# nju-websoft/OpenEA

Hardware: AMD Instinct MI355X
Metric: training triples/sec (k=10 truncated negatives + limited loss + Adagrad) (higher is better)
Workload: dtype f32; 1 GPU; BootEA/AlignE translational step, EN-FR-100K-V1 shape (synthetic), dim=100, GLOBAL batch=20000 positives (weak scaling: 20000 per GPU x 1 GPU), k=10, truncated eps=0.98; the same workload at every N (; global_batch=20000, entities=200000, parallelism=single

## Files before the change

### openea_amd/csrc/triple_step.hip

```cpp
#include <stdlib.h>

#include <algorithm>
#include <vector>

#include "common.h"
#include "step_plan.h"

namespace {

using oea::group_sum;

using oea::flag_t;
using oea::grad_t;

struct StepWs {
    grad_t *ent_grad, *rel_grad;
    grad_t *rel_extra;
    int64_t rel_copy_stride;
    flag_t *ent_touched, *rel_touched;
    grad_t *nrm_grad, *nrm_extra;
    flag_t *nrm_touched;
    double *partials;
    __device__ __forceinline__ grad_t *rel_copy(int64_t c) const {
        return c == 0 ? rel_grad : rel_extra + (c - 1) * rel_copy_stride;
    }
    __device__ __forceinline__ grad_t *nrm_copy(int64_t c) const {
        return c == 0 ? nrm_grad : nrm_extra + (c - 1) * rel_copy_stride;
    }
};
constexpr int kMaxBlocks = 4096;
constexpr int kRelCopies = 16;

static size_t align256(size_t x) { return (x + 255) / 256 * 256; }

static size_t ws_layout(int64_t n_ent, int64_t n_rel, int32_t ld, void *base, StepWs *ws) {
    size_t off = 0;
    char *b = static_cast<char *>(base);
    auto take = [&](size_t bytes) { size_t o = off; off += align256(bytes); return b ? b + o : nullptr; };
    grad_t *eg = (grad_t *)take(sizeof(grad_t) * (size_t)n_ent * ld);
    grad_t *rg = (grad_t *)take(sizeof(grad_t) * (size_t)n_rel * ld);
    grad_t *ng = (grad_t *)take(sizeof(grad_t) * (size_t)n_rel * ld);
    flag_t *et = (flag_t *)take(sizeof(flag_t) * (size_t)n_ent);
    flag_t *rt = (flag_t *)take(sizeof(flag_t) * (size_t)n_rel);
    flag_t *nt = (flag_t *)take(sizeof(flag_t) * (size_t)n_rel);
    grad_t *rx = (grad_t *)take(sizeof(grad_t) * (size_t)n_rel * ld * (kRelCopies - 1));
    grad_t *nx = (grad_t *)take(sizeof(grad_t) * (size_t)n_rel * ld * (kRelCopies - 1));
    double *pp = (double *)take(sizeof(double) * kMaxBlocks);
    if (ws) {
        ws->rel_copy_stride = n_rel * (int64_t)ld; ws->ent_grad = eg; ws->rel_grad = rg; ws->rel_extra = rx;
        ws->ent_touched = et; ws->rel_touched = rt; ws->nrm_grad = ng; ws->nrm_extra = nx; ws->nrm_touched = nt; ws->partials = pp;
    }
    return off;
}

template <int G, int IT>
struct Row {
    float v[IT];
};

template <int G, int IT, bool TIGHT = false>
__device__ __forceinline__ void load_row(const float *__restrict__ base, int ld, int lane, Row<G, IT> &r) {
#pragma unroll
    for (int it = 0; it < IT; ++it) {
        const int c = it * G + lane;
        r.v[it] = ((TIGHT && G == 32 && it < IT - 1) || c < ld) ? base[c] : 0.f;
    }
}
template <int G, int IT>
__device__ __forceinline__ void load_grad_raw(const grad_t *__restrict__ base, int ld, int lane, grad_t (&q)[IT]) {
#pragma unroll
    for (int it = 0; it < IT; ++it) {
        const int c = it * G + lane;
        q[it] = c < ld ? base[c] : (grad_t)0;
    }
}
template <int G, int IT>
__device__ __forceinline__ void load_grad_row(const grad_t *__restrict__ base, int ld, int lane, Row<G, IT> &r) {
#pragma unroll
    for (int it = 0; it < IT; ++it) {
        const int c = it * G + lane;
        r.v[it] = c < ld ? oea::grad_val(base[c]) : 0.f;
    }
}
template <int G, int IT>
__device__ __forceinline__ float sumsq(const Row<G, IT> &r) {
    float s = 0.f;
#pragma unroll
    for (int it = 0; it < IT; ++it) s += r.v[it] * r.v[it];
    return group_sum<G>(s);
}
template <int G, int IT>
__device__ __forceinline__ void normalize(Row<G, IT> &r, int on) {
    if (!on) return;
    const float inv = rsqrtf(fmaxf(sumsq<G, IT>(r), 1e-12f));
#pragma unroll
    for (int it = 0; it < IT; ++it) r.v[it] *= inv;
}
template <int G, int IT>
__device__ __forceinline__ float score(const Row<G, IT> &yh, const Row<G, IT> &yr, const Row<G, IT> &yt, int l1,
                                       Row<G, IT> &delta) {
    float s = 0.f;
#pragma unroll
    for (int it = 0; it < IT; ++it) {
        const float d = yh.v[it] + yr.v[it] - yt.v[it];
        delta.v[it] = d;
        s += l1 ? fabsf(d) : d * d;
    }
    return group_sum<G>(s);
}
__device__ __forceinline__ float sgn(float x) { return x > 0.f ? 1.f : (x < 0.f ? -1.f : 0.f); }

template <int G, int IT>
__device__ __forceinline__ void dscore(const Row<G, IT> &delta, float coef, int l1, Row<G, IT> &g) {
#pragma unroll
    for (int it = 0; it < IT; ++it) g.v[it] = l1 ? coef * sgn(delta.v[it]) : 2.f * coef * delta.v[it];
}
template <int G, int IT, bool SKIPZERO = true>
__device__ __forceinline__ void atomic_row(grad_t *__restrict__ dst, int ld, int lane, const Row<G, IT> &g, float sign) {
#pragma unroll
    for (int it = 0; it < IT; ++it) {
        const int c = it * G + lane;
        const float v = sign * g.v[it];
        if (((G == 32 && it < IT - 1) || c < ld) && (!SKIPZERO || v != 0.f)) oea::grad_add(dst + c, v);
    }
}

__device__ __forceinline__ float softplusf_(float x) { return x > 0.f ? x + log1pf(expf(-x)) : log1pf(expf(x)); }
__device__ __forceinline__ float sigmoidf_(float x) { return 1.f / (1.f + expf(-x)); }

__device__ __forceinline__ void triple_coef_kind(int loss_kind, const oea_step_cfg &cfg, bool is_pos, float s, float &coef,
                                                 float &l) {
    coef = 0.f; l = 0.f;
    switch (loss_kind) {
    case OEA_LOSS_LIMITED:
        if (is_pos) { const float x = s - cfg.pos_margin; if (x > 0.f) { l = x; coef = 1.f; } }
        else { const float x = cfg.neg_margin - s; if (x > 0.f) { l = cfg.balance * x; coef = -cfg.balance; } }
        break;
    case OEA_LOSS_LOGISTIC:
        if (is_pos) { l = softplusf_(s); coef = sigmoidf_(s); }
        else { l = softplusf_(-s); coef = -sigmoidf_(-s); }
        break;
    case OEA_LOSS_POSITIVE:
        l = s; coef = 1.f;
        break;
    case OEA_LOSS_ALIGN:
        l = softplusf_(s); coef = sigmoidf_(s);
        break;
    default: break;
    }
}
__device__ __forceinline__ void triple_coef(const oea_step_cfg &cfg, bool is_pos, float s, float &coef, float &l) {
    triple_coef_kind(cfg.loss_kind, cfg, is_pos, s, coef, l);
}

__device__ __forceinline__ void block_loss_partial(double loss_local, double *partials) {
// ... 283 lines not shown
    const float c_neg = L1 ? -cfg.balance : -2.f * cfg.balance;
    double loss_local = 0.0;
    for (int64_t p = w0; p < n_pos; p += nw) {
        const int32_t *pp = pos + 3 * p;
        const int32_t *ng = neg + p * k * 3;
        const int h = pp[0], r = pp[1], t = pp[2];
        Row<G, IT> yh, yr, yt;
        wave_load_row<IT>(rs_ent, h * row_b, v4, vt, yh);
        wave_load_row<IT>(rs_rel, r * row_b, v4, vt, yr);
        wave_load_row<IT>(rs_ent, t * row_b, v4, vt, yt);
        int ids[3 * KC];
        if (KT == KC || k == KC) {
#pragma unroll
            for (int q = 0; q < 3 * KC; ++q) ids[q] = ng[q];
        } else {
#pragma unroll
            for (int q = 0; q < 3 * KC; ++q) ids[q] = q < 3 * k ? ng[q] : 0;
        }
        unsigned bad = 0, xh = 0, xt = 0;
#pragma unroll
        for (int j = 0; j < KC; ++j)
            if (KT == KC || j < k) {
                const unsigned a = (unsigned)(ids[3 * j] ^ h), b = (unsigned)(ids[3 * j + 2] ^ t), c = (unsigned)(ids[3 * j + 1] ^ r);
                bad |= c | min(a, b);
                xh |= a;
                xt |= b;
            }
        if (bad | min(xh, xt)) {
            double ls = score_independent<G, IT>(ent, rel, ld, lane, p, h, r, t, true, cfg, ws, OEA_LOSS_LIMITED, L1);
#pragma unroll 1
            for (int j = 0; j < k; ++j)
                ls += score_independent<G, IT>(ent, rel, ld, lane, p, ng[3 * j], ng[3 * j + 1], ng[3 * j + 2], false, cfg, ws, OEA_LOSS_LIMITED, L1);
            loss_local += ls;
            continue;
        }
        const bool tails = xh == 0;
        int ce[KC];
        Row<G, IT> yc[KC];
#pragma unroll
        for (int j = 0; j < KC; ++j)
            if (KT == KC || j < k) {
                ce[j] = tails ? ids[3 * j + 2] : ids[3 * j];
                wave_load_row<IT>(rs_ent, ce[j] * row_b, v4, vt, yc[j]);
            }
        wave_normalize<IT>(yh);
        wave_normalize<IT>(yr);
        wave_normalize<IT>(yt);
        Row<G, IT> u, gacc, gpos;
        float sp = 0.f;
#pragma unroll
        for (int it = 0; it < IT; ++it) {
            u.v[it] = yh.v[it] + yr.v[it];
            const float d = u.v[it] - yt.v[it];
            gpos.v[it] = d;
            sp += L1 ? fabsf(d) : d * d;
        }
        const float xp = oea::wave_sum_uniform(sp) - cfg.pos_margin;
        const bool cpos = xp > 0.f;
        float lsum = cpos ? xp : 0.f;
#pragma unroll
        for (int it = 0; it < IT; ++it) {
            gpos.v[it] = cpos ? (L1 ? sgn(gpos.v[it]) : 2.f * gpos.v[it]) : 0.f;
            gacc.v[it] = gpos.v[it];
        }
        float sc[KC];
        if (tails) {
#pragma unroll
            for (int j = 0; j < KC; ++j)
                if (KT == KC || j < k) {
                    wave_normalize<IT>(yc[j]);
                    float s = 0.f;
#pragma unroll
                    for (int it = 0; it < IT; ++it) {
                        const float d = u.v[it] - yc[j].v[it];
                        yc[j].v[it] = d;
                        s += L1 ? fabsf(d) : d * d;
                    }
                    sc[j] = oea::wave_sum_uniform(s);
                }
        } else {
#pragma unroll
            for (int j = 0; j < KC; ++j)
                if (KT == KC || j < k) {
                    wave_normalize<IT>(yc[j]);
                    float s = 0.f;
#pragma unroll
                    for (int it = 0; it < IT; ++it) {
                        const float d = yc[j].v[it] + yr.v[it] - yt.v[it];
                        yc[j].v[it] = d;
                        s += L1 ? fabsf(d) : d * d;
                    }
                    sc[j] = oea::wave_sum_uniform(s);
                }
        }
        bool anyneg = false;
        const float sign_c = tails ? -1.f : 1.f;
#pragma unroll
        for (int j = 0; j < KC; ++j)
            if (KT == KC || j < k) {
                const float xn = cfg.neg_margin - sc[j];
                if (xn > 0.f) {
                    lsum += cfg.balance * xn;
                    anyneg = true;
                    Row<G, IT> g;
#pragma unroll
                    for (int it = 0; it < IT; ++it) {
                        g.v[it] = L1 ? c_neg * sgn(yc[j].v[it]) : c_neg * yc[j].v[it];
                        gacc.v[it] += g.v[it];
                    }
                    wave_atomic_row<IT>(rs_eg, ce[j] * row_g, vg, vgt, g, sign_c);
                    buf_flag_set(rs_et, ce[j]);
                }
            }
        if (PLAN) {
            const __amdgpu_buffer_rsrc_t rs_cb = __builtin_amdgcn_make_buffer_rsrc(contrib, 0, kBufRecords, kBufFlags);
            const int so = (int)p * 2 * row_b;
#pragma unroll
            for (int it = 0; it < IT; ++it) {
                const int vo = it < IT - 1 ? v4 + it * 256 : vt;
                __builtin_amdgcn_raw_buffer_store_b32(__builtin_bit_cast(unsigned, gacc.v[it]), rs_cb, vo, so, 0);
                __builtin_amdgcn_raw_buffer_store_b32(__builtin_bit_cast(unsigned, gpos.v[it]), rs_cb, vo, so + row_b, 0);
            }
        }
        if (cpos | anyneg) {
            const int copy = (int)(p % kRelCopies);
            grad_t *rgb = copy == 0 ? ws.rel_grad : ws.rel_extra + (copy - 1) * ws.rel_copy_stride;
            const __amdgpu_buffer_rsrc_t rs_rg = __builtin_amdgcn_make_buffer_rsrc(rgb, 0, (dbg & 1) ? 0 : kBufRecords, kBufFlags);
            const __amdgpu_buffer_rsrc_t rs_rt = __builtin_amdgcn_make_buffer_rsrc(ws.rel_touched, 0, (dbg & 4) ? 0 : kBufRecords, kBufFlags);
            wave_atomic_row<IT>(rs_rg, r * row_g, vg, vgt, gacc, 1.f);
            buf_flag_set(rs_rt, r);
            const unsigned via_atomics = PLAN ? pflags[p] : 3u;
            const bool h_full = tails, t_full = !tails;
            if ((via_atomics & 1u) && (h_full || cpos)) {
                wave_atomic_row<IT>(rs_eg, h * row_g, vg, vgt, h_full ? gacc : gpos, 1.f);
                buf_flag_set(rs_et, h);
            }
            if ((via_atomics & 2u) && (t_full || cpos)) {
                wave_atomic_row<IT>(rs_eg, t * row_g, vg, vgt, t_full ? gacc : gpos, -1.f);
                buf_flag_set(rs_et, t);
            }
        }
        loss_local += (double)lsum;
    }
    __shared__ double sred[8];
    if (lane == 0) sred[wv] = loss_local;
    __syncthreads();
    if (threadIdx.x == 0) {
        double s = 0.0;
        for (int w = 0; w < wpb; ++w) s += sred[w];
        ws.partials[blockIdx.x] = s;
    }
}

template <int G, int IT>
__device__ __forceinline__ float dot(const Row<G, IT> &a, const Row<G, IT> &b) {
    float s = 0.f;
#pragma unroll
    for (int it = 0; it < IT; ++it) s += a.v[it] * b.v[it];
    return group_sum<G>(s);
}
template <int G, int IT>
__device__ __forceinline__ void load_normal(const float *__restrict__ nrm, int r, int ld, int lane, Row<G, IT> &yn) {
    load_row<G, IT>(nrm + (int64_t)r * ld, ld, lane, yn);
    normalize<G, IT>(yn, 1);
    normalize<G, IT>(yn, 1);
}
template <int G, int IT>
__device__ double transh_independent(const float *__restrict__ ent, const float *__restrict__ rel, int ld, int lane,
                                     int64_t item, int h, int r, int t, bool is_pos, const oea_step_cfg &cfg,
                                     const StepWs &ws) {
    Row<G, IT> yh, yr, yt, yn, delta, g;
    load_row<G, IT>(ent + (int64_t)h * ld, ld, lane, yh);
    load_row<G, IT>(rel + (int64_t)r * ld, ld, lane, yr);
    load_row<G, IT>(ent + (int64_t)t * ld, ld, lane, yt);
    load_normal<G, IT>(cfg.normal, r, ld, lane, yn);
    normalize<G, IT>(yh, cfg.ent_l2_norm);
    normalize<G, IT>(yr, cfg.rel_l2_norm);
    normalize<G, IT>(yt, cfg.ent_l2_norm);
    const float ah = dot<G, IT>(yh, yn), at = dot<G, IT>(yt, yn);
    float s = 0.f;
#pragma unroll
    for (int it = 0; it < IT; ++it) {
        const float d = (yh.v[it] - ah * yn.v[it]) + yr.v[it] - (yt.v[it] - at * yn.v[it]);
        delta.v[it] = d;
        s += cfg.l1 ? fabsf(d) : d * d;
    }
    s = group_sum<G>(s);
    float coef, l;
    triple_coef(cfg, is_pos, s, coef, l);
    if (coef != 0.f) {
        dscore<G, IT>(delta, coef, cfg.l1, g);
        const float gdn = dot<G, IT>(g, yn);
        Row<G, IT> pg, gn;
#pragma unroll
        for (int it = 0; it < IT; ++it) {
            pg.v[it] = g.v[it] - gdn * yn.v[it];
            gn.v[it] = (at - ah) * g.v[it] + gdn * (yt.v[it] - yh.v[it]);
        }
        atomic_row<G, IT>(ws.ent_grad + (int64_t)h * ld, ld, lane, pg, 1.f);
        atomic_row<G, IT>(ws.ent_grad + (int64_t)t * ld, ld, lane, pg, -1.f);
        atomic_row<G, IT>(ws.rel_copy(item % kRelCopies) + (int64_t)r * ld, ld, lane, g, 1.f);
        atomic_row<G, IT>(ws.nrm_copy(item % kRelCopies) + (int64_t)r * ld, ld, lane, gn, 1.f);
        if (lane == 0) { ws.ent_touched[h] = 1.f; ws.ent_touched[t] = 1.f; ws.rel_touched[r] = 1.f; ws.nrm_touched[r] = 1.f; }
    }
    return (double)l;
}

template <int G, int IT>
__global__ __launch_bounds__(256) void triple_transh_grouped(
    const float *__restrict__ ent, const float *__restrict__ rel, int ld, const int32_t *__restrict__ pos,
    int64_t n_pos, const int32_t *__restrict__ neg, int k, oea_step_cfg cfg, StepWs ws) {
    const int lane = threadIdx.x % G;
    const int64_t grp = ((int64_t)blockIdx.x * blockDim.x + threadIdx.x) / G;
    const int64_t ngrp = (int64_t)gridDim.x * blockDim.x / G;
    double loss_local = 0.0;
    for (int64_t p = grp; p < n_pos; p += ngrp) {
        const int h = pos[3 * p], r = pos[3 * p + 1], t = pos[3 * p + 2];
        const int32_t *ng = neg + (int64_t)p * k * 3;
        Row<G, IT> yh, yr, yt, yn, ph, pt, g, gh, gr, gt, gn;
        load_row<G, IT>(ent + (int64_t)h * ld, ld, lane, yh);
        load_row<G, IT>(rel + (int64_t)r * ld, ld, lane, yr);
        load_row<G, IT>(ent + (int64_t)t * ld, ld, lane, yt);
        load_normal<G, IT>(cfg.normal, r, ld, lane, yn);
        normalize<G, IT>(yh, cfg.ent_l2_norm);
        normalize<G, IT>(yr, cfg.rel_l2_norm);
        normalize<G, IT>(yt, cfg.ent_l2_norm);
        const float ah = dot<G, IT>(yh, yn), at = dot<G, IT>(yt, yn);
        float s = 0.f;
#pragma unroll
        for (int it = 0; it < IT; ++it) {
            ph.v[it] = yh.v[it] - ah * yn.v[it];
            pt.v[it] = yt.v[it] - at * yn.v[it];
            const float d = ph.v[it] + yr.v[it] - pt.v[it];
            g.v[it] = d;
            s += cfg.l1 ? fabsf(d) : d * d;
        }
        s = group_sum<G>(s);
        float coef, l;
        triple_coef(cfg, true, s, coef, l);
        double lsum = (double)l;
        bool any = coef != 0.f;
        {
            Row<G, IT> d0 = g;
            dscore<G, IT>(d0, coef, cfg.l1, g);
            const float gdn = dot<G, IT>(g, yn);
#pragma unroll
            for (int it = 0; it < IT; ++it) {
                const float pg = g.v[it] - gdn * yn.v[it];
                gh.v[it] = pg; gt.v[it] = -pg; gr.v[it] = g.v[it];
                gn.v[it] = (at - ah) * g.v[it] + gdn * (yt.v[it] - yh.v[it]);
            }
        }
        for (int j0 = 0; j0 < k; j0 += 2) {
            int ch[2], cr[2], ct[2];
            Row<G, IT> yc[2];
#pragma unroll
            for (int u = 0; u < 2; ++u) {
                const int j = j0 + u < k ? j0 + u : j0;
                ch[u] = ng[3 * j]; cr[u] = ng[3 * j + 1]; ct[u] = ng[3 * j + 2];
                load_row<G, IT>(ent + (int64_t)((ch[u] == h) ? ct[u] : ch[u]) * ld, ld, lane, yc[u]);
            }
#pragma unroll
            for (int u = 0; u < 2; ++u) {
                if (j0 + u >= k) continue;
                const bool tail = ch[u] == h;
                if (!(cr[u] == r && (tail || ct[u] == t))) {
                    lsum += transh_independent<G, IT>(ent, rel, ld, lane, p, ch[u], cr[u], ct[u], false, cfg, ws);
                    continue;
                }
                const int ce = tail ? ct[u] : ch[u];
                normalize<G, IT>(yc[u], cfg.ent_l2_norm);
                const float ac = dot<G, IT>(yc[u], yn);
                Row<G, IT> delta;
                s = 0.f;
#pragma unroll
                for (int it = 0; it < IT; ++it) {
                    const float pc = yc[u].v[it] - ac * yn.v[it];
                    const float d = tail ? ph.v[it] + yr.v[it] - pc : pc + yr.v[it] - pt.v[it];
                    delta.v[it] = d;
                    s += cfg.l1 ? fabsf(d) : d * d;
                }
                s = group_sum<G>(s);
                triple_coef(cfg, false, s, coef, l);
                lsum += (double)l;
                if (coef == 0.f) continue;
                any = true;
                dscore<G, IT>(delta, coef, cfg.l1, g);
                const float gdn = dot<G, IT>(g, yn);
                Row<G, IT> pg;
#pragma unroll
                for (int it = 0; it < IT; ++it) {
                    pg.v[it] = g.v[it] - gdn * yn.v[it];
                    gr.v[it] += g.v[it];
                    if (tail) {
                        gh.v[it] += pg.v[it];
                        gn.v[it] += (ac - ah) * g.v[it] + gdn * (yc[u].v[it] - yh.v[it]);
                    } else {
                        gt.v[it] -= pg.v[it];
                        gn.v[it] += (at - ac) * g.v[it] + gdn * (yt.v[it] - yc[u].v[it]);
                    }
                }
                atomic_row<G, IT>(ws.ent_grad + (int64_t)ce * ld, ld, lane, pg, tail ? -1.f : 1.f);
                if (lane == 0) ws.ent_touched[ce] = 1.f;
            }
        }
        if (any) {
// ... 875 lines not shown
                bits &= bits - 1;
                if (at < g.cap) out[at] = w * 32 + b;
                ++at;
            }
            __syncthreads();
            if (tid == 0) s_base += chunk_total;
            __syncthreads();
        }
        if (tid == 0) counts[(int64_t)sr * g.world + o] = s_base - start;
    }
    if (tid == 0 && s_base > g.cap) atomicMax(err, 1);
}

__device__ __forceinline__ int halo_peer_of(const int32_t *__restrict__ pfx, int world, int64_t q) {
    int a = 0, b = world;
    while (b - a > 1) { const int m = (a + b) >> 1; if (pfx[m] <= q) a = m; else b = m; }
    return a;
}

template <int G, int IT>
__global__ __launch_bounds__(256) void halo_push_pack_kernel(StepWs ws, int ld, HaloGeom g, const int32_t *__restrict__ list ,
                                                             const int32_t *__restrict__ pfx ,
                                                             grad_t *__restrict__ send) {
    const int lane = threadIdx.x % G;
    const int64_t grp = ((int64_t)blockIdx.x * blockDim.x + threadIdx.x) / G, ngrp = (int64_t)gridDim.x * blockDim.x / G;
    const int64_t total = pfx[g.world];
    for (int64_t q = grp; q < total; q += ngrp) {
        const int o = halo_peer_of(pfx, g.world, q);
        if (o == g.rank) continue;
        const int64_t id = (int64_t)list[q] * g.world + o;
        const flag_t f = ws.ent_touched[id];
        grad_t *dst = send + q * (ld + 1);
#pragma unroll
        for (int it = 0; it < IT; ++it) {
            const int c = it * G + lane;
            if (c < ld) {
                dst[c] = f != 0 ? ws.ent_grad[id * ld + c] : (grad_t)0;
                if (f != 0) ws.ent_grad[id * ld + c] = 0;
            }
        }
        if (lane == 0) { dst[ld] = f; if (f != 0) ws.ent_touched[id] = 0; }
    }
}

template <int G, int IT>
__global__ __launch_bounds__(256) void halo_push_unpack_kernel(StepWs ws, int ld, HaloGeom g, const int32_t *__restrict__ lists_s ,
                                                               const int32_t *__restrict__ own_off ,
                                                               const int32_t *__restrict__ rpfx ,
                                                               const grad_t *__restrict__ recv) {
    const int lane = threadIdx.x % G;
    const int64_t grp = ((int64_t)blockIdx.x * blockDim.x + threadIdx.x) / G, ngrp = (int64_t)gridDim.x * blockDim.x / G;
    const int64_t total = rpfx[g.world];
    for (int64_t q = grp; q < total; q += ngrp) {
        const int r = halo_peer_of(rpfx, g.world, q);
        const int64_t j = lists_s[(int64_t)r * g.cap + own_off[r] + (q - rpfx[r])];
        const int64_t id = j * g.world + g.rank;
        const grad_t *src = recv + q * (ld + 1);
        if (src[ld] == 0) continue;
#pragma unroll
        for (int it = 0; it < IT; ++it) {
            const int c = it * G + lane;
            if (c < ld) { const grad_t v = src[c]; if (v != 0) oea::grad_add_raw(ws.ent_grad + id * ld + c, v); }
        }
        if (lane == 0) ws.ent_touched[id] = 1;
    }
}

template <int G, int IT>
__global__ __launch_bounds__(256) void halo_apply_kernel(float *__restrict__ ent, float *__restrict__ acc_own, int64_t n_ent,
                                                         float *__restrict__ rel, float *__restrict__ rel_acc, int64_t n_rel,
                                                         int ld, int world, int rank, int64_t rpr, grad_t *__restrict__ rel_x,
                                                         oea_step_cfg cfg, StepWs ws, int n_partials, double *__restrict__ loss_accum) {
    const int lane = threadIdx.x % G;
    const int64_t grp = ((int64_t)blockIdx.x * blockDim.x + threadIdx.x) / G;
    const int64_t ngrp = (int64_t)gridDim.x * blockDim.x / G;
    for (int64_t w = grp; w < rpr + n_rel; w += ngrp) {
        Row<G, IT> rv, rg, ra;
        if (w >= rpr) {
            const int64_t r = w - rpr;
            if (rel_x[n_rel * ld + r] == 0) continue;
            load_row<G, IT>(rel + r * ld, ld, lane, rv);
            load_grad_row<G, IT>(rel_x + r * ld, ld, lane, rg);
            if (cfg.opt_kind == OEA_OPT_ADAGRAD) load_row<G, IT>(rel_acc + r * ld, ld, lane, ra);
            flag_t dummy;
            apply_one_row<G, IT>(rel + r * ld, rel_acc + r * ld, rel_x + r * ld, &dummy, ld, lane, cfg.rel_l2_norm, cfg, rv, rg, ra);
            continue;
        }
        const int64_t j = w, id = j * world + rank;
        if (id >= n_ent || ws.ent_touched[id] == 0) continue;
        float *v = ent + id * ld;
        load_row<G, IT>(v, ld, lane, rv);
        load_grad_row<G, IT>(ws.ent_grad + id * ld, ld, lane, rg);
        if (cfg.opt_kind == OEA_OPT_ADAGRAD) load_row<G, IT>(acc_own + j * ld, ld, lane, ra);
        apply_one_row<G, IT>(v, acc_own + j * ld, ws.ent_grad + id * ld, ws.ent_touched + id, ld, lane, cfg.ent_l2_norm, cfg, rv, rg, ra);
    }
    if (blockIdx.x == 0 && threadIdx.x < 64) {
        double s = 0.0;
        for (int i = threadIdx.x; i < n_partials; i += 64) s += ws.partials[i];
        s = oea::wave_sum_d(s);
        if (threadIdx.x == 0) *loss_accum += s;
    }
}

__global__ void halo_rel_pack_kernel(StepWs ws, int64_t n_rel, int ld, grad_t *__restrict__ rel_x) {
    const int64_t total = n_rel * ld;
    for (int64_t i = (int64_t)blockIdx.x * blockDim.x + threadIdx.x; i < total; i += (int64_t)gridDim.x * blockDim.x) {
        const int64_t r = i / ld;
        const flag_t f = ws.rel_touched[r];
        rel_x[i] = f != 0 ? ws.rel_grad[i] : (grad_t)0;
        if (f != 0) ws.rel_grad[i] = 0;
    }
}
__global__ void halo_rel_flags_kernel(StepWs ws, int64_t n_rel, int ld, grad_t *__restrict__ rel_x) {
    const int64_t r = (int64_t)blockIdx.x * blockDim.x + threadIdx.x;
    if (r < n_rel) { rel_x[n_rel * ld + r] = ws.rel_touched[r]; ws.rel_touched[r] = 0; }
}

template <bool PACK>
__global__ void halo_pull_kernel(float *__restrict__ ent, int ld, HaloGeom g, const int32_t *__restrict__ lists_s ,
                                 const int32_t *__restrict__ own_off, const int32_t *__restrict__ pfx, float *__restrict__ buf) {
    const int cpr = ld / 4;
    const int64_t total = (int64_t)pfx[g.world] * cpr;
    for (int64_t i = (int64_t)blockIdx.x * blockDim.x + threadIdx.x; i < total; i += (int64_t)gridDim.x * blockDim.x) {
        const int64_t q = i / cpr;
        const int c = (int)(i - q * cpr);
        const int peer = halo_peer_of(pfx, g.world, q);
        if (peer == g.rank) continue;
        if (PACK) {
            const int64_t j = lists_s[(int64_t)peer * g.cap + own_off[peer] + (q - pfx[peer])];
            oea::st4(buf + q * ld + 4 * c, oea::ld4(ent + (j * g.world + g.rank) * ld + 4 * c));
        } else {
            const int64_t j = lists_s[q];
            oea::st4(ent + (j * g.world + peer) * ld + 4 * c, oea::ld4(buf + q * ld + 4 * c));
        }
    }
}

__global__ void halo_owned_rows_kernel(const float *__restrict__ ent, int64_t n_ent, int ld, int world, int rank, int64_t rpr,
                                       float *__restrict__ upd) {
    const int cpr = ld / 4;
    const int64_t total = rpr * cpr;
    for (int64_t i = (int64_t)blockIdx.x * blockDim.x + threadIdx.x; i < total; i += (int64_t)gridDim.x * blockDim.x) {
        const int64_t j = i / cpr, id = j * world + rank;
        const int c = (int)(i - j * cpr);
        oea::st4(upd + j * ld + 4 * c, id < n_ent ? oea::ld4(ent + id * ld + 4 * c) : make_float4(0.f, 0.f, 0.f, 0.f));
    }
}

static bool step_wave_enabled() {
    static const int env = [] { const char *e = getenv("OEA_STEP_WAVE"); return e ? atoi(e) : 1; }();
    return env != 0;
}

template <int IT64>
void launch_wave(int nb, int block, hipStream_t st, const float *ent, const float *rel, int ld, const int32_t *pos,
                 int64_t n_pos, const int32_t *neg, const oea_step_cfg &cfg, const StepWs &ws, float *contrib = nullptr,
                 const uint32_t *pflags = nullptr) {
    const int k = cfg.neg_group_k;
    static const int dbg = [] { const char *e = getenv("OEA_STEP_WAVE_DBG"); return e ? atoi(e) : 0; }();
#define OEA_WAVE(L1, KT)                                                                                                               \
    do {                                                                                                                               \
        if (contrib) oea::launch_timed(triple_wave<IT64, L1, KT, true>, nb, block, st, ent, rel, ld, pos, n_pos, neg, k, cfg, ws, dbg, contrib, pflags);   \
        else oea::launch_timed(triple_wave<IT64, L1, KT, false>, nb, block, st, ent, rel, ld, pos, n_pos, neg, k, cfg, ws, dbg, contrib, pflags);          \
    } while (0)
    if (k == 10) { if (cfg.l1) OEA_WAVE(1, 10); else OEA_WAVE(0, 10); }
    else { if (cfg.l1) OEA_WAVE(1, 0); else OEA_WAVE(0, 0); }
#undef OEA_WAVE
}

static bool step_runtime_kind() {
    static const int env = [] { const char *e = getenv("OEA_STEP_RUNTIME_KIND"); return e ? atoi(e) : 0; }();
    return env != 0;
}

static bool wave_rule(const oea_step_cfg &cfg, int64_t n_ent, int64_t n_rel, int32_t ld) {
    return cfg.score_kind == OEA_SCORE_TRANSE && cfg.loss_kind == OEA_LOSS_LIMITED && cfg.ent_l2_norm && cfg.rel_l2_norm &&
           cfg.neg_group_k >= 1 && cfg.neg_group_k <= 10 && ld <= 256 &&
           std::max(n_ent, n_rel) * (int64_t)ld * (int64_t)sizeof(grad_t) < ((int64_t)1 << 30) && step_wave_enabled() &&
           !step_runtime_kind();
}

template <int G, int IT>
void launch_grouped(int nb, int block, hipStream_t st, const float *ent, const float *rel, int ld, const int32_t *pos,
                    int64_t n_pos, const int32_t *neg, const oea_step_cfg &cfg, const StepWs &ws, bool wave, float *contrib = nullptr,
                    const uint32_t *pflags = nullptr) {
    const bool runtime_kind = step_runtime_kind();
    const int k = cfg.neg_group_k;
    if constexpr ((G == 32 && IT <= 4) || (G == 64 && IT == 4)) {
        if (wave) {
            constexpr int IT64 = G == 32 ? (IT + 1) / 2 : 4;
            static const int blk_env = [] { const char *e = getenv("OEA_STEP_WAVE_BLOCK"); return e ? atoi(e) : 0; }();
            const int wblock = G == 32 ? (blk_env == 256 || blk_env == 512 ? blk_env : 512) : (block / G) * 64;
            launch_wave<IT64>(nb, wblock, st, ent, rel, ld, pos, n_pos, neg, cfg, ws, contrib, pflags);
            return;
        }
    }
#define OEA_GROUPED(LOSS, L1) oea::launch_timed(triple_grouped<G, IT, LOSS, L1>, nb, block, st, ent, rel, ld, pos, n_pos, neg, k, cfg, ws)
    if (runtime_kind) OEA_GROUPED(-1, -1);
    else if (cfg.loss_kind == OEA_LOSS_LIMITED) { if (cfg.l1) OEA_GROUPED(OEA_LOSS_LIMITED, 1); else OEA_GROUPED(OEA_LOSS_LIMITED, 0); }
    else if (cfg.loss_kind == OEA_LOSS_LOGISTIC) { if (cfg.l1) OEA_GROUPED(OEA_LOSS_LOGISTIC, 1); else OEA_GROUPED(OEA_LOSS_LOGISTIC, 0); }
    else if (cfg.loss_kind == OEA_LOSS_POSITIVE) { if (cfg.l1) OEA_GROUPED(OEA_LOSS_POSITIVE, 1); else OEA_GROUPED(OEA_LOSS_POSITIVE, 0); }
    else OEA_GROUPED(-1, -1);
#undef OEA_GROUPED
}

static bool apply_g16(int64_t n_ent, int64_t n_rel, int32_t ld) {
    static const int env_g16 = [] { const char *e = getenv("OEA_APPLY_G16"); return e ? atoi(e) : -1; }();
    return env_g16 >= 0 ? env_g16 != 0 : (n_ent + n_rel) * (int64_t)ld * 12 > (int64_t)128 << 20;
}

static int64_t step_items(const oea_step_cfg &cfg, int64_t n_pos, int64_t n_neg) {
    const bool transh = cfg.score_kind == OEA_SCORE_TRANSH, transd = cfg.score_kind == OEA_SCORE_TRANSD;
    const bool transh_grouped = transh && cfg.loss_kind != OEA_LOSS_MARGIN && (n_neg == 0 || cfg.neg_group_k > 0);
    const bool projected = transd || (transh && !transh_grouped);
    const bool grouped = transh_grouped || (!projected && cfg.neg_group_k > 0 && cfg.loss_kind != OEA_LOSS_MARGIN);
    return (grouped || cfg.loss_kind == OEA_LOSS_MARGIN) ? n_pos : n_pos + n_neg;
}

template <int G, int IT>
int launch_step(float *ent, float *ent_acc, int64_t n_ent, float *rel, float *rel_acc, int64_t n_rel,
                int32_t ld, const int32_t *pos, int64_t n_pos, const int32_t *neg, int64_t n_neg,
                const oea_step_cfg &cfg, const StepWs &ws, double *loss_accum, int phase, hipStream_t st,
                const oea::StepPlanView *plan = nullptr, int plan_step = 0, int64_t plan_first_pos = 0) {
    const int block = 256, gpb = block / G;
    const bool transh = cfg.score_kind == OEA_SCORE_TRANSH, transd = cfg.score_kind == OEA_SCORE_TRANSD;
    const bool dense_opt = cfg.opt_kind == OEA_OPT_ADAM || cfg.opt_kind == OEA_OPT_ADADELTA;
    const bool transh_grouped = transh && cfg.loss_kind != OEA_LOSS_MARGIN && (n_neg == 0 || cfg.neg_group_k > 0);
    const bool projected = transd || (transh && !transh_grouped);
    const bool grouped = transh_grouped || (!projected && cfg.neg_group_k > 0 && cfg.loss_kind != OEA_LOSS_MARGIN);
    const int64_t items = step_items(cfg, n_pos, n_neg);
    const int nb1 = (int)std::min<int64_t>(std::max<int64_t>(oea::ceil_div(items, gpb), 1), kMaxBlocks);
    if (phase != OEA_PHASE_APPLY) {
        oea::prof_call();
        if (transd)
            oea::launch_timed(triple_projected<G, IT, OEA_SCORE_TRANSD>, nb1, block, st, ent, rel, ld, pos, n_pos, neg, n_neg, cfg, ws);
        else if (projected)
            oea::launch_timed(triple_projected<G, IT, OEA_SCORE_TRANSH>, nb1, block, st, ent, rel, ld, pos, n_pos, neg, n_neg, cfg, ws);
        else if (transh)
            oea::launch_timed(triple_transh_grouped<G, IT>, nb1, block, st, ent, rel, ld, pos, n_pos, neg, n_neg ? cfg.neg_group_k : 0, cfg, ws);
        else if (grouped)
            launch_grouped<G, IT>(nb1, block, st, ent, rel, ld, pos, n_pos, neg, cfg, ws, wave_rule(cfg, n_ent, n_rel, ld),
                                  plan ? plan->contrib : nullptr, plan ? plan->pflags + plan_first_pos : nullptr);
        else
            oea::launch_timed(triple_generic<G, IT>, nb1, block, st, ent, rel, ld, pos, n_pos, neg, n_neg, cfg, ws);
        if (phase == OEA_PHASE_GRAD || dense_opt)
            fold_rel_copies_kernel<<<(unsigned)std::min<int64_t>(oea::ceil_div(n_rel * (int64_t)ld, 256), 1024), 256, 0, st>>>(
                ws, n_rel * (int64_t)ld, transh ? 1 : 0);
    }
    const int nb2 = (int)std::min<int64_t>(std::max<int64_t>(oea::ceil_div(n_ent + n_rel, gpb), 1), 16384);
    if (phase != OEA_PHASE_GRAD) {
        hipEvent_t ev0 = nullptr, ev1 = nullptr;
        (void)oea::prof_pair(&ev0, &ev1);
        if (dense_opt) {
            const double t = (double)cfg.opt_t;
            const float lr_t = cfg.opt_kind == OEA_OPT_ADAM
                                   ? (float)((double)cfg.lr * std::sqrt(1.0 - std::pow((double)cfg.beta2, t)) / (1.0 - std::pow((double)cfg.beta1, t)))
                                   : cfg.lr;
            oea::launch_events(apply_rows_dense<G, IT>, nb2, block, st, ev0, ev1, ent, ent_acc, n_ent, rel, rel_acc, n_rel, ld, cfg, ws,
                              items > 0 ? nb1 : 0, loss_accum, lr_t);
        } else {
            static const int env_r = [] { const char *e = getenv("OEA_APPLY_ROWS"); return e ? atoi(e) : 0; }();
            const int R = env_r ? env_r : 1;
            const int n_part = items > 0 ? nb1 : 0;
            const int folded = phase == OEA_PHASE_APPLY;
            static const int flag_first_env = [] { const char *e = getenv("OEA_APPLY_FLAG_FIRST"); return e ? atoi(e) : 0; }();
            const int flag_first = plan ? 1 : flag_first_env;
            auto nb = [&](int r) { return (int)std::min<int64_t>(std::max<int64_t>(oea::ceil_div(n_rel + oea::ceil_div(n_ent, r), gpb), 1), 16384); };
            const bool g16 = apply_g16(n_ent, n_rel, ld);
            if (plan) {
                static_assert(kMaxBlocks <= 16 * 256, "the partials block reads 16 per lane");
                const int64_t bound = 2 * n_pos;
                if (g16 && G == 32) {
                    const int it16 = (ld + 15) / 16;
                    const int relb = (int)std::max<int64_t>(oea::ceil_div(n_rel, 16), 1);
                    const int planb = (int)std::min<int64_t>(std::max<int64_t>(oea::ceil_div(bound, 16), 1), 8192);
                    const int scanb = (int)std::min<int64_t>(std::max<int64_t>(oea::ceil_div(n_ent, 256), 1), 4096);
#ifndef OEA_DET_SCRATCH
                    static const bool v4 = [] { const char *e = getenv("OEA_APPLY_V4"); return !(e && e[0] == '0'); }();
#define OEA_APPLYP16(ITX) do { if (v4) oea::launch_events(apply_step_plan_v4<16, ITX>, relb + planb + scanb + 1, block, st, ev0, ev1, ent, ent_acc, n_ent, rel, rel_acc, n_rel, ld, cfg, ws, n_part, loss_accum, folded, relb, scanb, plan->recs, plan->vals_b, plan->step_first, plan_step, plan->inplan, plan->contrib); \
    else oea::launch_events(apply_step_plan<16, ITX>, relb + planb + scanb + 1, block, st, ev0, ev1, ent, ent_acc, n_ent, rel, rel_acc, n_rel, ld, cfg, ws, n_part, loss_accum, folded, relb, scanb, plan->recs, plan->vals_b, plan->step_first, plan_step, plan->inplan, plan->contrib); } while (0)
#else
#define OEA_APPLYP16(ITX) oea::launch_events(apply_step_plan<16, ITX>, relb + planb + scanb + 1, block, st, ev0, ev1, ent, ent_acc, n_ent, rel, rel_acc, n_rel, ld, cfg, ws, n_part, loss_accum, folded, relb, scanb, plan->recs, plan->vals_b, plan->step_first, plan_step, plan->inplan, plan->contrib)
#endif
                    if (it16 <= 2) OEA_APPLYP16(2);
                    else if (it16 <= 4) OEA_APPLYP16(4);
                    else if (it16 == 5) OEA_APPLYP16(5);
                    else if (it16 == 6) OEA_APPLYP16(6);
                    else if (it16 == 7) OEA_APPLYP16(7);
                    else OEA_APPLYP16(8);
#undef OEA_APPLYP16
                } else {
                    const int relb = (int)std::max<int64_t>(oea::ceil_div(n_rel, gpb), 1);
                    const int planb = (int)std::min<int64_t>(std::max<int64_t>(oea::ceil_div(bound, gpb), 1), 8192);
                    const int scanb = (int)std::min<int64_t>(std::max<int64_t>(oea::ceil_div(n_ent, 256), 1), 4096);
                    oea::launch_events(apply_step_plan<G, IT>, relb + planb + scanb + 1, block, st, ev0, ev1, ent, ent_acc, n_ent, rel, rel_acc,
                                       n_rel, ld, cfg, ws, n_part, loss_accum, folded, relb, scanb, plan->recs, plan->vals_b,
                                       plan->step_first, plan_step, plan->inplan, plan->contrib);
                }
            } else
            if (g16 && G == 32 && R == 1) {
                const int it16 = (ld + 15) / 16;
                const int nbg = (int)std::min<int64_t>(std::max<int64_t>(oea::ceil_div(n_rel + n_ent, 16), 1), 16384);
#define OEA_APPLY16(ITX) oea::launch_events(apply_rows<16, ITX, 1>, nbg, block, st, ev0, ev1, ent, ent_acc, n_ent, rel, rel_acc, n_rel, ld, cfg, ws, n_part, loss_accum, folded, flag_first)
                if (it16 <= 2) OEA_APPLY16(2);
                else if (it16 <= 4) OEA_APPLY16(4);
                else if (it16 == 5) OEA_APPLY16(5);
                else if (it16 == 6) OEA_APPLY16(6);
                else if (it16 == 7) OEA_APPLY16(7);
                else OEA_APPLY16(8);
#undef OEA_APPLY16
            } else
            if (R >= 4 && IT <= 4)
                oea::launch_events(apply_rows<G, IT, 4>, nb(4), block, st, ev0, ev1, ent, ent_acc, n_ent, rel, rel_acc, n_rel, ld, cfg, ws, n_part, loss_accum, folded, flag_first);
            else if (R >= 2 && IT <= 8)
                oea::launch_events(apply_rows<G, IT, 2>, nb(2), block, st, ev0, ev1, ent, ent_acc, n_ent, rel, rel_acc, n_rel, ld, cfg, ws, n_part, loss_accum, folded, flag_first);
            else
                oea::launch_events(apply_rows<G, IT, 1>, nb(1), block, st, ev0, ev1, ent, ent_acc, n_ent, rel, rel_acc, n_rel, ld, cfg, ws, n_part, loss_accum, folded, flag_first);
        }
        if (transh)
            apply_normal_rows<G, IT><<<(unsigned)std::max<int64_t>(oea::ceil_div(n_rel, gpb), 1), block, 0, st>>>(
// ... 680 lines not shown
```

Before: 257.6 million triples/s.

## Add persistent software-pipelined wave kernel prefetching ids and rows ahead

Adds a persistent-grid variant of the per-positive wave kernel. Each wave loops over positives with a stride of the grid size and prefetches the next positive's embedding rows and the id tuple two iterations ahead, hiding gather latency behind scoring. It is launched only when the number of positives exceeds the resident wave slots, with the grid sized by an occupancy query cached per device, and it zeroes the unused loss partials. The cost is higher register pressure from holding two sets of 13 rows, which may lower occupancy.

```diff
diff --git a/openea_amd/csrc/triple_step.hip b/openea_amd/csrc/triple_step.hip
--- a/openea_amd/csrc/triple_step.hip
+++ b/openea_amd/csrc/triple_step.hip
@@ -1,6 +1,7 @@
 #include <stdlib.h>
 
 #include <algorithm>
+#include <atomic>
 #include <vector>
 
 #include "common.h"
@@ -590,6 +591,250 @@
     }
 }
 
+constexpr int kWaveK = 10;
+
+struct WaveIds {
+    int h, r, t, ce[kWaveK];
+    bool tails, outside;
+};
+template <int IT>
+struct WaveRows {
+    Row<64, IT> yh, yr, yt, yc[kWaveK];
+};
+struct WaveCtx {
+    __amdgpu_buffer_rsrc_t rs_ent, rs_rel, rs_eg, rs_et;
+    int v4, vt, vg, vgt, row_b, row_g;
+};
+
+template <int KT>
+__device__ __forceinline__ void wave_classify(const int (&ids)[3 * kWaveK], int k, WaveIds &w) {
+    constexpr int KC = kWaveK;
+    unsigned bad = 0, xh = 0, xt = 0;
+#pragma unroll
+    for (int j = 0; j < KC; ++j)
+        if (KT == KC || j < k) {
+            const unsigned a = (unsigned)(ids[3 * j] ^ w.h), b = (unsigned)(ids[3 * j + 2] ^ w.t), c = (unsigned)(ids[3 * j + 1] ^ w.r);
+            bad |= c | min(a, b);
+            xh |= a;
+            xt |= b;
+        }
+    w.outside = (bad | min(xh, xt)) != 0;
+    w.tails = xh == 0;
+}
+template <int IT, int KT>
+__device__ __forceinline__ void wave_request_rows(const WaveCtx &c, const WaveIds &w, int k, WaveRows<IT> &rows) {
+    wave_load_row<IT>(c.rs_ent, w.h * c.row_b, c.v4, c.vt, rows.yh);
+    wave_load_row<IT>(c.rs_rel, w.r * c.row_b, c.v4, c.vt, rows.yr);
+    wave_load_row<IT>(c.rs_ent, w.t * c.row_b, c.v4, c.vt, rows.yt);
+#pragma unroll
+    for (int j = 0; j < kWaveK; ++j)
+        if (KT == kWaveK || j < k) wave_load_row<IT>(c.rs_ent, w.ce[j] * c.row_b, c.v4, c.vt, rows.yc[j]);
+}
+
+template <int IT, int L1, int KT, bool PLAN>
+__device__ __forceinline__ float wave_score_positive(const WaveCtx &c, const WaveIds &w, WaveRows<IT> &rows, int64_t p, int k,
+                                                     const oea_step_cfg &cfg, const StepWs &ws, int dbg, float c_neg,
+                                                     float *__restrict__ contrib, const uint32_t *__restrict__ pflags) {
+    constexpr int G = 64, KC = kWaveK;
+    Row<G, IT> &yh = rows.yh, &yr = rows.yr, &yt = rows.yt;
+    Row<G, IT>(&yc)[KC] = rows.yc;
+    const int h = w.h, r = w.r, t = w.t;
+    const bool tails = w.tails;
+    const int v4 = c.v4, vt = c.vt, vg = c.vg, vgt = c.vgt, row_b = c.row_b, row_g = c.row_g;
+    wave_normalize<IT>(yh);
+    wave_normalize<IT>(yr);
+    wave_normalize<IT>(yt);
+    Row<G, IT> u, gacc, gpos;
+    float sp = 0.f;
+#pragma unroll
+    for (int it = 0; it < IT; ++it) {
+        u.v[it] = yh.v[it] + yr.v[it];
+        const float d = u.v[it] - yt.v[it];
+        gpos.v[it] = d;
+        sp += L1 ? fabsf(d) : d * d;
+    }
+    const float xp = oea::wave_sum_uniform(sp) - cfg.pos_margin;
+    const bool cpos = xp > 0.f;
+    float lsum = cpos ? xp : 0.f;
+#pragma unroll
+    for (int it = 0; it < IT; ++it) {
+        gpos.v[it] = cpos ? (L1 ? sgn(gpos.v[it]) : 2.f * gpos.v[it]) : 0.f;
+        gacc.v[it] = gpos.v[it];
+    }
+    float sc[KC];
+    if (tails) {
+#pragma unroll
+        for (int j = 0; j < KC; ++j)
+            if (KT == KC || j < k) {
+                wave_normalize<IT>(yc[j]);
+                float s = 0.f;
+#pragma unroll
+                for (int it = 0; it < IT; ++it) {
+                    const float d = u.v[it] - yc[j].v[it];
+                    yc[j].v[it] = d;
+                    s += L1 ? fabsf(d) : d * d;
+                }
+                sc[j] = oea::wave_sum_uniform(s);
+            }
+    } else {
+#pragma unroll
+        for (int j = 0; j < KC; ++j)
+            if (KT == KC || j < k) {
+                wave_normalize<IT>(yc[j]);
+                float s = 0.f;
+#pragma unroll
+                for (int it = 0; it < IT; ++it) {
+                    const float d = yc[j].v[it] + yr.v[it] - yt.v[it];
+                    yc[j].v[it] = d;
+                    s += L1 ? fabsf(d) : d * d;
+                }
+                sc[j] = oea::wave_sum_uniform(s);
+            }
+    }
+    bool anyneg = false;
+    const float sign_c = tails ? -1.f : 1.f;
+#pragma unroll
+    for (int j = 0; j < KC; ++j)
+        if (KT == KC || j < k) {
+            const float xn = cfg.neg_margin - sc[j];
+            if (xn > 0.f) {
+                lsum += cfg.balance * xn;
+                anyneg = true;
+                Row<G, IT> g;
+#pragma unroll
+                for (int it = 0; it < IT; ++it) {
+                    g.v[it] = L1 ? c_neg * sgn(yc[j].v[it]) : c_neg * yc[j].v[it];
+                    gacc.v[it] += g.v[it];
+                }
+                wave_atomic_row<IT>(c.rs_eg, w.ce[j] * row_g, vg, vgt, g, sign_c);
+                buf_flag_set(c.rs_et, w.ce[j]);
+            }
+        }
+    if (PLAN) {
+        const __amdgpu_buffer_rsrc_t rs_cb = __builtin_amdgcn_make_buffer_rsrc(contrib, 0, kBufRecords, kBufFlags);
+        const int so = (int)p * 2 * row_b;
+#pragma unroll
+        for (int it = 0; it < IT; ++it) {
+            const int vo = it < IT - 1 ? v4 + it * 256 : vt;
+            __builtin_amdgcn_raw_buffer_store_b32(__builtin_bit_cast(unsigned, gacc.v[it]), rs_cb, vo, so, 0);
+            __builtin_amdgcn_raw_buffer_store_b32(__builtin_bit_cast(unsigned, gpos.v[it]), rs_cb, vo, so + row_b, 0);
+        }
+    }
+    if (cpos | anyneg) {
+        const int copy = (int)(p % kRelCopies);
+        grad_t *rgb = copy == 0 ? ws.rel_grad : ws.rel_extra + (copy - 1) * ws.rel_copy_stride;
+        const __amdgpu_buffer_rsrc_t rs_rg = __builtin_amdgcn_make_buffer_rsrc(rgb, 0, (dbg & 1) ? 0 : kBufRecords, kBufFlags);
+        const __amdgpu_buffer_rsrc_t rs_rt = __builtin_amdgcn_make_buffer_rsrc(ws.rel_touched, 0, (dbg & 4) ? 0 : kBufRecords, kBufFlags);
+        wave_atomic_row<IT>(rs_rg, r * row_g, vg, vgt, gacc, 1.f);
+        buf_flag_set(rs_rt, r);
+        const unsigned via_atomics = PLAN ? pflags[p] : 3u;
+        const bool h_full = tails, t_full = !tails;
+        if ((via_atomics & 1u) && (h_full || cpos)) {
+            wave_atomic_row<IT>(c.rs_eg, h * row_g, vg, vgt, h_full ? gacc : gpos, 1.f);
+            buf_flag_set(c.rs_et, h);
+        }
+        if ((via_atomics & 2u) && (t_full || cpos)) {
+            wave_atomic_row<IT>(c.rs_eg, t * row_g, vg, vgt, t_full ? gacc : gpos, -1.f);
+            buf_flag_set(c.rs_et, t);
+        }
+    }
+    return lsum;
+}
+template <int IT, int L1>
+__device__ __forceinline__ double wave_score_outside(const float *__restrict__ ent, const float *__restrict__ rel, int ld, int lane,
+                                                     int64_t p, int h, int r, int t, const int32_t *__restrict__ ng, int k,
+                                                     const oea_step_cfg &cfg, const StepWs &ws) {
+    double ls = score_independent<64, IT>(ent, rel, ld, lane, p, h, r, t, true, cfg, ws, OEA_LOSS_LIMITED, L1);
+#pragma unroll 1
+    for (int j = 0; j < k; ++j)
+        ls += score_independent<64, IT>(ent, rel, ld, lane, p, ng[3 * j], ng[3 * j + 1], ng[3 * j + 2], false, cfg, ws, OEA_LOSS_LIMITED, L1);
+    return ls;
+}
+
+__device__ __forceinline__ int wave_request_ids(const int32_t *__restrict__ pos, const int32_t *__restrict__ neg, int64_t p, int k,
+                                                int lane) {
+    const bool lo = lane < 32;
+    const int32_t *src = lo ? neg + p * k * 3 + lane : pos + 3 * p + (lane - 32);
+    return (lo ? lane < 3 * k : lane < 35) ? *src : 0;
+}
+template <int KT>
+__device__ __forceinline__ void wave_decode_ids(int idv, int k, WaveIds &w) {
+    int ids[3 * kWaveK];
+#pragma unroll
+    for (int q = 0; q < 3 * kWaveK; ++q) ids[q] = __builtin_amdgcn_readlane(idv, q);
+    w.h = __builtin_amdgcn_readlane(idv, 32);
+    w.r = __builtin_amdgcn_readlane(idv, 33);
+    w.t = __builtin_amdgcn_readlane(idv, 34);
+    wave_classify<KT>(ids, k, w);
+#pragma unroll
+    for (int j = 0; j < kWaveK; ++j) w.ce[j] = w.tails ? ids[3 * j + 2] : ids[3 * j];
+}
+
+template <int IT, int L1, int KT, bool PLAN>
+__global__ __launch_bounds__(256, (IT <= 2 ? 4 : 2)) void triple_wave_pipe(
+    const float *__restrict__ ent, const float *__restrict__ rel, int ld, const int32_t *__restrict__ pos,
+    int64_t n_pos, const int32_t *__restrict__ neg, int k, oea_step_cfg cfg, StepWs ws, int dbg, float *__restrict__ contrib,
+    const uint32_t *__restrict__ pflags, int n_part) {
+    if (KT > 0) k = KT;
+    const int lane = threadIdx.x & 63;
+    const int wv = __builtin_amdgcn_readfirstlane((int)(threadIdx.x >> 6));
+    const int wpb = blockDim.x >> 6;
+    const int64_t w0 = (int64_t)blockIdx.x * wpb + wv, nw = (int64_t)gridDim.x * wpb;
+    WaveCtx c;
+    c.row_b = ld * 4, c.row_g = ld << kGradShift;
+    c.rs_ent = __builtin_amdgcn_make_buffer_rsrc(const_cast<float *>(ent), 0, (dbg & 2) ? 0 : kBufRecords, kBufFlags);
+    c.rs_rel = __builtin_amdgcn_make_buffer_rsrc(const_cast<float *>(rel), 0, (dbg & 2) ? 0 : kBufRecords, kBufFlags);
+    c.rs_eg = __builtin_amdgcn_make_buffer_rsrc(ws.ent_grad, 0, (dbg & 1) ? 0 : kBufRecords, kBufFlags);
+    c.rs_et = __builtin_amdgcn_make_buffer_rsrc(ws.ent_touched, 0, (dbg & 4) ? 0 : kBufRecords, kBufFlags);
+    c.v4 = lane * 4, c.vg = lane << kGradShift;
+    const int c_last = (IT - 1) * 64 + lane;
+    c.vt = c_last < ld ? c_last * 4 : kBufOob, c.vgt = c_last < ld ? c_last << kGradShift : kBufOob;
+    const float c_neg = L1 ? -cfg.balance : -2.f * cfg.balance;
+    double loss_local = 0.0;
+    WaveIds cur_w = {}, nxt_w = {};
+    WaveRows<IT> cur = {};
+    int idv = 0;
+    if (w0 < n_pos) {
+        const int idv0 = wave_request_ids(pos, neg, w0, k, lane);
+        if (w0 + nw < n_pos) idv = wave_request_ids(pos, neg, w0 + nw, k, lane);
+        wave_decode_ids<KT>(idv0, k, cur_w);
+        if (!cur_w.outside) wave_request_rows<IT, KT>(c, cur_w, k, cur);
+        if (w0 + nw < n_pos) {
+            wave_decode_ids<KT>(idv, k, nxt_w);
+            if (w0 + 2 * nw < n_pos) idv = wave_request_ids(pos, neg, w0 + 2 * nw, k, lane);
+        }
+    }
+    for (int64_t p = w0; p < n_pos; p += nw) {
+        WaveIds nn_w = {};
+        WaveRows<IT> nxt = {};
+        if (p + 2 * nw < n_pos && !nxt_w.outside) {
+            wave_request_rows<IT, KT>(c, nxt_w, k, nxt);
+            wave_decode_ids<KT>(idv, k, nn_w);
+        } else if (p + 2 * nw < n_pos) {
+            wave_decode_ids<KT>(idv, k, nn_w);
+        } else if (p + nw < n_pos && !nxt_w.outside) {
+            wave_request_rows<IT, KT>(c, nxt_w, k, nxt);
+        }
+        if (p + 3 * nw < n_pos) idv = wave_request_ids(pos, neg, p + 3 * nw, k, lane);
+        if (cur_w.outside)
+            loss_local += wave_score_outside<IT, L1>(ent, rel, ld, lane, p, cur_w.h, cur_w.r, cur_w.t, neg + p * k * 3, k, cfg, ws);
+        else
+            loss_local += (double)wave_score_positive<IT, L1, KT, PLAN>(c, cur_w, cur, p, k, cfg, ws, dbg, c_neg, contrib, pflags);
+        cur_w = nxt_w;
+        cur = nxt;
+        nxt_w = nn_w;
+    }
+    __shared__ double sred[8];
+    if (lane == 0) sred[wv] = loss_local;
+    __syncthreads();
+    if (threadIdx.x == 0) {
+        double s = 0.0;
+        for (int w = 0; w < wpb; ++w) s += sred[w];
+        ws.partials[blockIdx.x] = s;
+        for (int q = blockIdx.x + gridDim.x; q < n_part; q += gridDim.x) ws.partials[q] = 0.0;
+    }
+}
+
 template <int G, int IT>
 __device__ __forceinline__ float dot(const Row<G, IT> &a, const Row<G, IT> &b) {
     float s = 0.f;
@@ -1771,20 +2016,53 @@
     return env != 0;
 }
 
+template <auto Kernel>
+int resident_blocks(int block) {
+    constexpr int kDevices = 64;
+    static std::atomic<int> cache[kDevices][2];
+    int dev = 0;
+    if (hipGetDevice(&dev) != hipSuccess || dev < 0 || dev >= kDevices) dev = 0;
+    std::atomic<int> &slot = cache[dev][block == 512];
+    int v = slot.load(std::memory_order_relaxed);
+    if (v == 0) {
+        int per_cu = 0, cus = 0;
+        if (hipOccupancyMaxActiveBlocksPerMultiprocessor(&per_cu, Kernel, block, 0) != hipSuccess) per_cu = 1;
+        if (hipDeviceGetAttribute(&cus, hipDeviceAttributeMultiprocessorCount, dev) != hipSuccess) cus = 1;
+        v = std::max(per_cu, 1) * std::max(cus, 1);
+        slot.store(v, std::memory_order_relaxed);
+    }
+    return v;
+}
+
 template <int IT64>
 void launch_wave(int nb, int block, hipStream_t st, const float *ent, const float *rel, int ld, const int32_t *pos,
                  int64_t n_pos, const int32_t *neg, const oea_step_cfg &cfg, const StepWs &ws, float *contrib = nullptr,
                  const uint32_t *pflags = nullptr) {
     const int k = cfg.neg_group_k;
     static const int dbg = [] { const char *e = getenv("OEA_STEP_WAVE_DBG"); return e ? atoi(e) : 0; }();
+    static const int grid_cap = [] { const char *e = getenv("OEA_STEP_WAVE_GRID"); return e ? atoi(e) : 0; }();
+#define OEA_WAVE_P(L1, KT, PLAN)                                                                                                       \
+    do {                                                                                                                               \
+        const int64_t slots = (int64_t)resident_blocks<triple_wave<IT64, L1, KT, PLAN>>(block) * (block / 64);                  \
+        if (grid_cap > 0 || n_pos > slots) {                                                                                           \
+            int grid = std::min(nb, resident_blocks<triple_wave_pipe<IT64, L1, KT, PLAN>>(256));                                      \
+            if (grid_cap > 0) grid = std::min(grid, grid_cap);                                                                         \
+            oea::launch_timed(triple_wave_pipe<IT64, L1, KT, PLAN>, grid, 256, st, ent, rel, ld, pos, n_pos, neg, k, cfg, ws, dbg,    \
+                              contrib, pflags, nb);                                                                                    \
+        } else {                                                                                                                       \
+            oea::launch_timed(triple_wave<IT64, L1, KT, PLAN>, nb, block, st, ent, rel, ld, pos, n_pos, neg, k, cfg, ws, dbg,         \
+                              contrib, pflags);                                                                                        \
+        }                                                                                                                              \
+    } while (0)
 #define OEA_WAVE(L1, KT)                                                                                                               \
     do {                                                                                                                               \
-        if (contrib) oea::launch_timed(triple_wave<IT64, L1, KT, true>, nb, block, st, ent, rel, ld, pos, n_pos, neg, k, cfg, ws, dbg, contrib, pflags);   \
-        else oea::launch_timed(triple_wave<IT64, L1, KT, false>, nb, block, st, ent, rel, ld, pos, n_pos, neg, k, cfg, ws, dbg, contrib, pflags);          \
+        if (contrib) OEA_WAVE_P(L1, KT, true);                                                                                         \
+        else OEA_WAVE_P(L1, KT, false);                                                                                                \
     } while (0)
     if (k == 10) { if (cfg.l1) OEA_WAVE(1, 10); else OEA_WAVE(0, 10); }
     else { if (cfg.l1) OEA_WAVE(1, 0); else OEA_WAVE(0, 0); }
 #undef OEA_WAVE
+#undef OEA_WAVE_P
 }
 
 static bool step_runtime_kind() {
```

Result: slower. 251.7 million triples/s (-2.3%).
